# 2gunsu/monocon-pytorch

Measured on AMD Instinct MI355X. Metric: images/sec (384x1280) fwd+bwd, higher is better.
Workload: dtype f32 (f16x2); 1 GPU; train step B=32/GPU 3x384x1280 (configs[2] shape, fp32 values, mode f16x2); global_batch=32, parallelism=dp1, precision_mode=f16x2

## Files before the change

### monocon-pytorch_amd/csrc/mc_train_api.hip

```cpp
#include "mc_internal.h"

#include <algorithm>
#include <cmath>
#include <cstdlib>
#include <cstring>
#include <vector>

static int check_targets(mc_handle *h, const mc_targets *t, const char *who) {
    if (!t) return fail(h, "%s: targets is NULL", who);
    const void *p[] = {t->center_heatmap_target, t->wh_target, t->offset_target, t->dim_target, t->alpha_cls_target,
                       t->alpha_offset_target, t->depth_target, t->center2kpt_offset_target, t->kpt_heatmap_target,
                       t->kpt_heatmap_offset_target, t->indices, t->indices_kpt, t->mask_target,
                       t->mask_center2kpt_offset, t->mask_kpt_heatmap_offset};
    for (size_t i = 0; i < sizeof(p) / sizeof(p[0]); ++i)
        if (!p[i]) return fail(h, "%s: targets field %d is NULL", who, (int)i);
    return 0;
}

extern "C" {

int mc_make_targets(mc_handle *h, const mc_labels *lab, int B, int max_objs, int pad_h, int pad_w, int fh, int fw,
                    const mc_targets *t, void *stream) {
    if (!h) return -1;
    if (!lab || !lab->gt_bboxes || !lab->gt_labels || !lab->gt_bboxes_3d || !lab->depths || !lab->gt_kpts_2d ||
// ... 114 lines not shown
    HIPCHK(h, mc::launch_focal_grad(preds[0], t->center_heatmap_target, (size_t)B * 3 * HW, aux + 0, grad_losses, 0, dpreds[0], st, wrt_pred));
    HIPCHK(h, mc::launch_focal_grad(preds[1], t->kpt_heatmap_target, (size_t)B * 9 * HW, aux + 1, grad_losses, 5, dpreds[1], st, wrt_pred));
    mc::GatherLossArgs g{};
    fill_gather_args(g, preds, dpreds, t, B, max_objs, (int)HW, scratch_losses, aux + 2, grad_losses);
    g.wrt_pred = wrt_pred;
    g.partial = gather_ws(h);
    HIPCHK(h, mc::launch_gathered_losses(g, 1, st));
    return 0;
}

int mc_losses_backward(mc_handle *h, const float *const preds[MC_NUM_PREDS], const mc_targets *t, int B, int max_objs,
                       int fh, int fw, const float *grad_losses, float *const dpreds[MC_NUM_PREDS], void *stream) {
    return losses_backward_impl(h, preds, t, B, max_objs, fh, fw, grad_losses, dpreds, stream, 0);
}

int mc_losses_backward_pred(mc_handle *h, const float *const preds[MC_NUM_PREDS], const mc_targets *t, int B, int max_objs,
                            int fh, int fw, const float *grad_losses, float *const dpreds[MC_NUM_PREDS], void *stream) {
    return losses_backward_impl(h, preds, t, B, max_objs, fh, fw, grad_losses, dpreds, stream, 1);
}

int mc_op_conv_wgrad(mc_handle *h, const float *const src[], const int src_channels[], int nsrc, int B, int Hin, int Win,
                     const float *dy, int Cout, int ksize, int stride, float *dw_oihw, void *stream) {
    if (!h) return -1;
    if (!src || !src_channels || !dy || !dw_oihw || nsrc < 1 || nsrc > 4) return fail(h, "mc_op_conv_wgrad: bad argument");
    if (!((ksize == 3 && (stride == 1 || stride == 2)) || (ksize == 1 && stride == 1)))
        return fail(h, "mc_op_conv_wgrad: unsupported k=%d stride=%d", ksize, stride);
    if (Cout % 4) return fail(h, "mc_op_conv_wgrad: Cout must be a multiple of 4");
    HIPCHK(h, hipSetDevice(h->device));
    hipStream_t st = static_cast<hipStream_t>(stream);
    mc::WgradArgs a{};
    int cin = 0;
    for (int i = 0; i < nsrc; ++i) {
        if (!src[i] || src_channels[i] % 16) return fail(h, "mc_op_conv_wgrad: source %d needs C %% 16 == 0", i);
        a.src[i].p = src[i]; a.src[i].C = src_channels[i];
        cin += src_channels[i];
    }
    a.nsrc = nsrc; a.B = B; a.Hin = Hin; a.Win = Win;
    a.Hout = (Hin + 2 * (ksize / 2) - ksize) / stride + 1;
    a.Wout = (Win + 2 * (ksize / 2) - ksize) / stride + 1;
    a.Cin = cin; a.Cout = Cout; a.dy = dy; a.dy_ld = Cout;
    a.prec = h->prec;
    ScratchBuf slots;
    if (h->prec == 3) {
        HIPCHK(h, slots.alloc(5 * mc::AMAX_WORDS * sizeof(unsigned)));
        unsigned *sl = slots.as<unsigned>();
        HIPCHK(h, hipMemsetAsync(sl, 0, 5 * mc::AMAX_WORDS * sizeof(unsigned), st));
        for (int i = 0; i < nsrc; ++i) {
            HIPCHK(h, mc::launch_absmax(src[i], (size_t)B * Hin * Win * src_channels[i], sl + i * mc::AMAX_WORDS, st));
            a.amax_x[i] = sl + i * mc::AMAX_WORDS;
        }
        HIPCHK(h, mc::launch_absmax(dy, (size_t)B * a.Hout * a.Wout * Cout, sl + 4 * mc::AMAX_WORDS, st));
        a.amax_dy = sl + 4 * mc::AMAX_WORDS;
    }
    mc::wgrad_plan(a, ksize, stride);
    void *part = nullptr;
    HIPCHK(h, hipMalloc(&part, mc::wgrad_partial_floats(a, ksize) * sizeof(float)));
    a.partial = static_cast<float *>(part);
    hipError_t e = mc::launch_wgrad(a, ksize, stride, dw_oihw, st);
    hipError_t e2 = hipStreamSynchronize(st);
    (void)hipFree(part);
    HIPCHK(h, e);
    HIPCHK(h, e2);
    return 0;
}

int mc_op_conv_dgrad(mc_handle *h, const float *dy, const float *weight_oihw, int B, int Hin, int Win, int CinTotal,
                     int c_off, int Cs, int Cout, int ksize, int stride, int accumulate, float *dx, void *stream) {
    if (!h) return -1;
    if (!dy || !weight_oihw || !dx) return fail(h, "mc_op_conv_dgrad: null argument");
    if (!((ksize == 3 && (stride == 1 || stride == 2)) || (ksize == 1 && stride == 1)))
        return fail(h, "mc_op_conv_dgrad: unsupported k=%d stride=%d", ksize, stride);
    if (Cout % 16 || Cs % 4 || c_off < 0 || c_off + Cs > CinTotal) return fail(h, "mc_op_conv_dgrad: bad channel arguments");
    if (stride == 2 && ((Hin | Win) & 1)) return fail(h, "mc_op_conv_dgrad: stride 2 needs even Hin, Win");
    HIPCHK(h, hipSetDevice(h->device));
    hipStream_t st = static_cast<hipStream_t>(stream);
    const int Ho = (Hin + 2 * (ksize / 2) - ksize) / stride + 1, Wo = (Win + 2 * (ksize / 2) - ksize) / stride + 1;
    const int CsP = mc::conv_coutp(Cs), pieces = h->prec == 2 ? 3 : (h->prec == 3 ? 2 : 1);
    const int nclass = stride == 2 ? 4 : 1;
    std::vector<void *> tmp;
    hipError_t e = hipSuccess;
    ScratchBuf slots;
    unsigned *sl = nullptr;
    if (h->prec == 3) {
        HIPCHK(h, slots.alloc((mc::AMAX_WORDS + 1) * sizeof(unsigned)));
        sl = slots.as<unsigned>();
        HIPCHK(h, hipMemsetAsync(sl, 0, (mc::AMAX_WORDS + 1) * sizeof(unsigned), st));
        HIPCHK(h, mc::launch_absmax(dy, (size_t)B * Ho * Wo * Cout, sl, st));
        HIPCHK(h, mc::launch_absmax(weight_oihw, (size_t)Cout * CinTotal * ksize * ksize, sl + mc::AMAX_WORDS, st, true));
    }
    for (int cls = 0; cls < nclass && e == hipSuccess; ++cls) {
        const int cid = stride == 2 ? cls : -1;
        const int py = cls >> 1, px = cls & 1;
        const int taps = stride == 2 ? (1 + py) * (1 + px) : ksize * ksize;
        const size_t pn = (size_t)taps * Cout * CsP;
        void *panel = nullptr, *panel16 = nullptr;
        if (hipMalloc(&panel, pn * 4) != hipSuccess) { e = hipErrorOutOfMemory; break; }
        tmp.push_back(panel);
        (void)hipMemsetAsync(panel, 0, pn * 4, st);
        e = mc::launch_pack_conv_w_dgrad(weight_oihw, Cout, CinTotal, ksize, c_off, Cs, CsP, Cout, cid, static_cast<float *>(panel), st);
        if (e != hipSuccess) break;
        if (h->prec >= 1 && Cout % 32 == 0) {
            if (hipMalloc(&panel16, pn * 2 * pieces) != hipSuccess) { e = hipErrorOutOfMemory; break; }
            tmp.push_back(panel16);
            (void)hipMemsetAsync(panel16, 0, pn * 2 * pieces, st);
            e = mc::launch_pack_conv_w_dgrad_bf16(weight_oihw, Cout, CinTotal, ksize, c_off, Cs, CsP, Cout, cid, pieces, panel16, st,
                                                  sl ? sl + mc::AMAX_WORDS : nullptr);
            if (e != hipSuccess) break;
        }
        mc::ConvArgs d{};
        d.nsrc = 1; d.src[0].p = dy; d.src[0].C = Cout;
// ... 81 lines not shown
```

### monocon-pytorch_amd/csrc/mc_train_plan.hip

```cpp
#include <atomic>
#include <deque>
#include <functional>

#include "mc_internal.h"

using namespace mc;

namespace {

using Fn = std::function<int(mc_handle *, hipStream_t)>;

struct PlanSwitches {
    long long lazy_z;
    long long lazy_min;
    long long lazy_feat;
    long long zbits;
    long long grad_pool;
    long long grad_pool_cool;
    long long head_dx_fuse;
    long long dgrad_s2_thin;
    long long stem_fuse;
    long long bm_epilogue;
    long long wres_bwd;
    long long dual_stream;
    int side_sync_lo = 0, side_sync_hi = 0;
    bool plan_debug = false;
};
const struct { const char *name; long long PlanSwitches::*field; long long def; } SWITCH_TABLE[] = {
    {"MONOCON_HIP_LAZY_Z", &PlanSwitches::lazy_z, 3},
    {"MONOCON_HIP_LAZY_MIN", &PlanSwitches::lazy_min, 900000},
    {"MONOCON_HIP_LAZY_FEAT", &PlanSwitches::lazy_feat, 0},
    {"MONOCON_HIP_ZBITS", &PlanSwitches::zbits, 1},
    {"MONOCON_HIP_GRAD_POOL", &PlanSwitches::grad_pool, 1},
    {"MONOCON_HIP_GRAD_POOL_COOL", &PlanSwitches::grad_pool_cool, 2},
    {"MONOCON_HIP_HEAD_DX_FUSE", &PlanSwitches::head_dx_fuse, 1},
    {"MONOCON_HIP_DGRAD_S2_THIN", &PlanSwitches::dgrad_s2_thin, 1},
    {"MONOCON_HIP_STEM_FUSE", &PlanSwitches::stem_fuse, 1},
    {"MONOCON_HIP_BM_EPILOGUE", &PlanSwitches::bm_epilogue, 1},
    {"MONOCON_HIP_WRES_BWD", &PlanSwitches::wres_bwd, 0},
    {"MONOCON_HIP_DUAL_STREAM", &PlanSwitches::dual_stream, 1},
};
PlanSwitches read_switches() {
    PlanSwitches sw{};
    std::string changed;
    for (const auto &d : SWITCH_TABLE) {
        const char *e = std::getenv(d.name);
        sw.*d.field = e ? std::atoll(e) : d.def;
        if (sw.*d.field != d.def) changed += std::string(" ") + d.name + "=" + std::to_string(sw.*d.field);
    }
    if (const char *e = std::getenv("MONOCON_HIP_SIDE_SYNC")) {
        if (std::sscanf(e, "%d:%d", &sw.side_sync_lo, &sw.side_sync_hi) != 2) sw.side_sync_lo = sw.side_sync_hi = 0;
        if (sw.side_sync_lo < sw.side_sync_hi) changed += std::string(" MONOCON_HIP_SIDE_SYNC=") + e;
    }
    sw.plan_debug = std::getenv("MONOCON_HIP_PLAN_DEBUG") != nullptr;
    if (sw.plan_debug && !changed.empty()) fprintf(stderr, "[plan] switches off their defaults:%s\n", changed.c_str());
    return sw;
}

struct PoolBwdArgs {
    const float *x, *dout, *la, *lb;
    float *dx, *stats;
    int B, H, W, C, acc;
};

struct LastWriter {
    enum Kind { NONE, DGRAD_CONV, POOL_BWD, DECONV_BWD } kind = NONE;
    union {
        ConvArgs *conv;
        PoolBwdArgs *pool;
        float **deconv_stats;
    };
    LastWriter() : conv(nullptr) {}
    LastWriter(ConvArgs *c) : kind(c ? DGRAD_CONV : NONE), conv(c) {}
    LastWriter(PoolBwdArgs *p) : kind(p ? POOL_BWD : NONE), pool(p) {}
    LastWriter(float **s) : kind(s ? DECONV_BWD : NONE), deconv_stats(s) {}
};

struct TNode {
    Tensor t;
    float *g = nullptr;
    bool ginit = false, needs_grad = true;
    LastWriter last;
    const float *la = nullptr, *lb = nullptr;
    bool lrelu = true;
};

struct PackJob {
    const float *w;
    int Cout, CinTotal, k, c_off, Cs, CsP, CoutPad;
    int cls;
    float *dst;
    void *dst16;
    unsigned *amax;
// ... 411 lines not shown
                    HIPCHK(hh, launch_dgrad_s2_thin(dyp, B, Hd, Wd, Cd, w_master, CinTotal, c_off, gp, acc, dmax, wmax, st));
                    return 0;
                });
                wrote(srcnode);
                return;
            }
            for (int cls = 0; cls < 4; ++cls) {
                const int py = cls >> 1, px = cls & 1;
                ConvArgs d = dgrad_conv(cls);
                const int ld = sn.t.C;
                d.out = sn.g + ((size_t)py * sn.t.W + px) * ld; d.out_ld = ld;
                d.o_px = 2 * ld; d.o_row = 2 * sn.t.W * ld; d.o_img = sn.t.H * sn.t.W * ld;
                if (sn.ginit) { d.res = d.out; d.res_ld = ld; d.r_px = d.o_px; d.r_row = d.o_row; d.r_img = d.o_img; }
                const int kcode = (1 + py) * 10 + (1 + px);
                const int kk = kcode == 11 ? 1 : kcode;
                d.cfg = ts->ok ? mc_choose_conv_cfg(h, d, kk, 1) : CFG_128x32;
                push_bwd([=](mc_handle *hh, hipStream_t st) { HIPCHK(hh, launch_conv(d, kk, 1, st)); return 0; });
            }
            wrote(srcnode);
            return;
        }
        ConvArgs d = dgrad_conv(-1);
        d.out = sn.g; d.out_ld = sn.t.C;
        if (sn.ginit) { d.res = sn.g; d.res_ld = sn.t.C; }
        if (dy.H != sn.t.H || dy.W != sn.t.W) { ts->ok = false; h->err = "train plan: dgrad shape mismatch"; }
        d.cfg = ts->ok ? mc_choose_conv_cfg(h, d, ks, 1) : CFG_128x32;
        if (sw.wres_bwd < 2) d.cfg &= ~CFG_WRES;
        ts->dgrads.push_back(d);
        ConvArgs *dp = &ts->dgrads.back();
        push_bwd([=](mc_handle *hh, hipStream_t st) { HIPCHK(hh, launch_conv(*dp, ks, 1, st)); return 0; });
        wrote(srcnode, (d.cfg == CFG_SMALL && !conv_thin_ok(d, ks, 1)) ? nullptr : dp);
    }

    int emit_wgrad(const std::vector<int> &srcs, const Tensor &dy, int dy_ld, int Cout, int ks, int stride, float *dw) {
        WgradArgs a{};
        a.nsrc = (int)srcs.size();
        auto fill = [&] {
            int cin = 0;
            for (int i = 0; i < a.nsrc; ++i) {
                fill_src(a.src[i], srcs[i]);
                a.amax_x[i] = ts->nodes[srcs[i]].t.amax;
                cin += a.src[i].C;
            }
            return cin;
        };
        for (int s_ : srcs)
            if (ts->nodes[s_].la && !ts->nodes[s_].lrelu) materialise(s_);
        int cin = fill();
        a.amax_dy = dy.amax;
        const Tensor &s0 = ts->nodes[srcs[0]].t;
        a.B = s0.B; a.Hin = s0.H; a.Win = s0.W; a.Hout = dy.H; a.Wout = dy.W; a.Cin = cin; a.Cout = Cout;
        a.dy = dy.p; a.dy_ld = dy_ld;
        a.prec = h->prec;
        wgrad_plan(a, ks, stride);
        bool any_lazy = false;
        for (int i = 0; i < a.nsrc; ++i) any_lazy |= a.src[i].la != nullptr;
        if (any_lazy && !wgrad_lazy_capable(a, ks, stride)) {
            for (int s_ : srcs) materialise(s_);
            fill();
        }
        a.partial = alloc(wgrad_partial_floats(a, ks));
        return push_bwd([=](mc_handle *hh, hipStream_t st) { HIPCHK(hh, launch_wgrad(a, ks, stride, dw, st)); return 0; }, ON_SIDE);
    }

    struct BnBwd { Tensor dy; float *coef; bool affine_skipped; };
    BnBwd bn_backward(const Rec &r, const std::string &bn, bool caller_forms_dy = false) {
        TNode &zn = ts->nodes[r.z];
        Tensor dy = r.y;
        dy.p = zn.g;
        dy.amax = slot();
        unsigned *dymax = dy.amax;
        const int B = r.y.B, C = r.y.C, rows = r.y.H * r.y.W;
        const float *yp = r.y.p, *gz = zn.g, *zp = zn.t.p, *gamma = P(bn + ".weight", C), *mean = r.mean, *rstd = r.rstd;
        float *dg = G(bn + ".weight", C), *db = G(bn + ".bias", C), *dyp = dy.p;
        float *coef = alloc((size_t)C * 4);
        const int relu = r.relu ? ((r.res < 0 && r.ca && r.cb) ? 2 : 1) : 0;
        const float *fa = r.ca, *fb = r.cb;
        float *gres = nullptr;
        int gmode = 0;
        if (r.res >= 0 && ts->nodes[r.res].needs_grad) {
            gres = g_acquire(r.res);
            gmode = ts->nodes[r.res].ginit ? 2 : 1;
            wrote(r.res);
        }
        const double n = (double)B * rows;
        auto step = [&](float *partial, int nbp, int cstride, bool reduce, bool affine) {
            double *fold = fold_scratch(nbp, C);
            const int arelu = reduce ? relu : 0;
            const float *aa = reduce ? fa : nullptr, *ab = reduce ? fb : nullptr;
            push_bwd([=](mc_handle *hh, hipStream_t st) {
                if (reduce) HIPCHK(hh, launch_chan_reduce(yp, gz, zp, nullptr, B, rows, C, 1, relu, partial, C, st, fa, fb));
                HIPCHK(hh, launch_bn_bwd_finalize(partial, nbp, cstride, n, C, gamma, mean, rstd, dg, db, coef, st, fold));
                if (affine)
                    HIPCHK(hh, launch_affine_bwd(gz, zp, yp, coef, B, (size_t)rows, C, 0, arelu, dyp, gres, gmode, st, aa, ab, nullptr,
                                                 nullptr, dymax));
                return 0;
            });
            return BnBwd{dy, coef, !affine};
        };
        const LastWriter last = zn.last;
        ConvArgs *lc = last.kind == LastWriter::DGRAD_CONV ? last.conv : nullptr;
        if (sw.bm_epilogue == 0 || (sw.bm_epilogue > 1 && r.y.H * r.y.W > sw.bm_epilogue)) lc = nullptr;
        if (sw.plan_debug)
            fprintf(stderr, "[plan] bn_backward %-40s %4d ch %4dx%-4d relu %d res %d last-writer-conv %d\n", bn.c_str(), C, r.y.H,
                    r.y.W, relu, r.res >= 0, lc != nullptr);
        if (lc && lc->out == zn.g && lc->Cout == C && lc->out_ld == C && lc->Hout == r.y.H && lc->Wout == r.y.W && !lc->stats) {
// ... 608 lines not shown
```

### monocon-pytorch_amd/csrc/train.h

```cpp
#pragma once
#include <hip/hip_runtime.h>
#include <stdint.h>
#include <vector>

#include "conv_mfma.h"

namespace mc {

struct TargetArgs {
    const float *gt_bboxes, *gt_labels, *gt_bboxes_3d, *depths, *gt_kpts_2d, *gt_kpts_valid, *mask;
    int B, max_objs, num_kpt, num_classes, fh, fw;
    float h_ratio, w_ratio;
    float *center_heatmap, *kpt_heatmap;
    float *wh, *offset, *dim, *alpha_cls, *alpha_offset, *depth, *c2k, *kho;
    long long *indices, *indices_kpt;
    uint8_t *mask_target;
    float *mask_c2k, *mask_kho;
};
hipError_t launch_make_targets(const TargetArgs &a, hipStream_t st);

hipError_t launch_focal(const float *p, const float *t, size_t n, float *partial, float *loss_out, float *aux,
                        hipStream_t st);
hipError_t launch_focal_grad(const float *p, const float *t, size_t n, const float *aux, const float *gscale, int gidx,
                             float *dlogit, hipStream_t st, int wrt_pred = 0);
// ... 104 lines not shown
                                const float *wpk, float *din,
                                float *stats = nullptr);

hipError_t launch_pack_conv_w_dgrad(const float *w, int Cout, int CinTotal, int k, int c_off, int Cs, int CsP, int CoutPad,
                                    int cls, float *dst, hipStream_t st);
hipError_t launch_dpred_pack(const float *const dpred[10], int ld, int B, int HW, float *out, hipStream_t st);
hipError_t launch_dpred_pack_user(const float *const dpred[10], const float *const pred[10], const float *const grad[10], int ld,
                                  int B, int HW, float *out, hipStream_t st);
struct AttnTrainArgs {
    const float *stats;
    int chunks, stat_ld, B, HW;
    double *stats64;
    float *rm[9], *rv[9];
    long long *nbt[9];
    const float *att_w[9], *att_g[9], *att_b[9];
    float *att_rm[9], *att_rv[9];
    long long *att_nbt[9];
    const float *weight_[9], *bias_[9];
    float *sv_inst;
    float *mu_r;
    float *bn10;
    float *that, *yatt;
    float *gamma_p;
    float *scale, *shift;
};
struct AttnGradPtrs { float *d_weight_[9], *d_bias_[9], *d_att_w[9], *d_att_g[9], *d_att_b[9]; };
hipError_t launch_attn_train_fwd(const AttnTrainArgs &a, hipStream_t st);
hipError_t launch_attn_train_bwd(const AttnTrainArgs &a, const float *partial, int rb_per_img, const AttnGradPtrs &gp,
                                 float *coef, hipStream_t st);
hipError_t launch_head_bwd(const float *draw, int ld, const float *z, const float *x, const float *w1, int B, int HW,
                           int blocks, float *d, float *dw_partial, float *red_partial, hipStream_t st,
                           const float *scale = nullptr, const float *shift = nullptr);
hipError_t launch_head_dx(const float *draw, int ld, const float *x, const float *w1, const float *coef, int B, int HW, int blocks,
                          float *dx, float *csum, float *csum_out, unsigned *amax, hipStream_t st, const float *scale,
                          const float *shift);
hipError_t launch_splitk_reduce(const float *partial, int ksplit, int T, int Cout, int Cin, float *dw, hipStream_t st);
int stem_wgrad_blocks(int B, int H, int W);
hipError_t launch_stem_wgrad(const float *img, const float *dy, int B, int H, int W, float *partial, float *dw,
                             hipStream_t st, const unsigned *img_amax = nullptr, const unsigned *dy_amax = nullptr,
                             const float *y = nullptr, const float *coef = nullptr, const unsigned *y_amax = nullptr);

struct WgradArgs {
    ConvSrc src[4];
    int nsrc;
    int B, Hin, Win, Hout, Wout, Cin, Cout;
    const float *dy;
    int dy_ld;
    float *partial;
    int ksplit, n_tiles, c_tiles, ppr, ppi, groups_per_img;
    int small;
    int prec;
    int pb;
    int pipe;
    const unsigned *amax_x[4], *amax_dy;
};
void wgrad_plan(WgradArgs &a, int ks, int stride);
size_t wgrad_partial_floats(const WgradArgs &a, int ks);
hipError_t launch_wgrad(const WgradArgs &a, int ks, int stride, float *dw_oihw, hipStream_t st);
bool wgrad_lazy_capable(const WgradArgs &a, int ks, int stride);
bool wgrad_bf16_ok(const WgradArgs &a, int ks, int stride);
hipError_t launch_wgrad_bf16(const WgradArgs &a, int ks, int stride, int WN, int WC, hipStream_t st);
int wgrad_bf16_patches(int prec);
int wgrad_pipe_tile(const WgradArgs &a, int ks, int stride);
void wgrad_pipe_plan(WgradArgs &a, int tile);
hipError_t launch_wgrad_pipe(const WgradArgs &a, int ks, hipStream_t st);
bool wgrad_thin_ok(const WgradArgs &a, int ks, int stride);
hipError_t launch_wgrad_thin(const WgradArgs &a, hipStream_t st);

}
```

### monocon-pytorch_amd/csrc/wgrad_mfma.hip

```cpp
#include <algorithm>
#include <cstdlib>
#include "conv_mfma.h"
#include "train.h"

namespace mc {

template <int KS, int S, int WN, int WC>
struct WgCfg {
    static constexpr int PB = 2;
    static constexpr int NB = 32 * WN, CB = 32 * WC;
    static constexpr int NT = 64 * WN * WC;
    static constexpr int PAD = KS / 2;
    static constexpr int IH = 3 * S + KS, IW = 7 * S + KS, NPIX = IH * IW;
    static constexpr int CBP = CB + 4, NBP = NB + 4;
    static constexpr int LDS_FLOATS = PB * NPIX * CBP + PB * 32 * NBP;
    static constexpr size_t LDS_BYTES = sizeof(float) * LDS_FLOATS;
};

template <int KS, int S, int WN, int WC>
__global__ __launch_bounds__(64 * WN * WC, 2) void wgrad_mfma_kernel(const WgradArgs a) {
    using Cfg = WgCfg<KS, S, WN, WC>;
    constexpr int PB = Cfg::PB, NB = Cfg::NB, CB = Cfg::CB, NT = Cfg::NT, PAD = Cfg::PAD;
    constexpr int IW = Cfg::IW, NPIX = Cfg::NPIX, CBP = Cfg::CBP, NBP = Cfg::NBP;
    constexpr int T = KS * KS;
// ... 282 lines not shown
    for (int e = tid; e < 9 * NTN * 4 * 64; e += 256) {
        const int l = e & 63, idx = e >> 6;
        const int q = idx & 3, nt = (idx >> 2) % NTN, t = (idx >> 2) / NTN;
        const int n = nt * 16 + 4 * (l >> 4) + q, c = l & 15;
        a.partial[(((size_t)blockIdx.x * 9 + t) * COUT + n) * CIN + c] = red[idx][l];
    }
}

static bool wgrad_is_small(const WgradArgs &a, int ks, int stride) {
    return ks == 3 && a.nsrc == 1 && a.Cin == 16 && (a.Cout == 16 || a.Cout == 32) && a.dy_ld == a.Cout &&
           (stride == 1 || stride == 2) && a.Wout % 4 == 0 && a.Wout >= 8 &&
           a.Hout == (a.Hin + 2 - 3) / stride + 1 && a.Wout == (a.Win + 2 - 3) / stride + 1;
}

template <int KS, int S, int WN, int WC>
static hipError_t launch_wg(WgradArgs a, hipStream_t st) {
    using Cfg = WgCfg<KS, S, WN, WC>;
    auto kern = wgrad_mfma_kernel<KS, S, WN, WC>;
    static DynLdsOnce attr_set;
    static const size_t lds_req = [] {
#ifdef MC_DEBUG_HOOKS
        const char *e = std::getenv("MONOCON_HIP_WGRAD_LDS_KB");
        const size_t pad = e ? (size_t)std::atoi(e) * 1024 : 0;
        return pad > Cfg::LDS_BYTES ? pad : (size_t)Cfg::LDS_BYTES;
#else
        return (size_t)Cfg::LDS_BYTES;
#endif
    }();
    {
        const hipError_t e = attr_set.ensure(reinterpret_cast<const void *>(kern), (int)(lds_req));
        if (e != hipSuccess) return e;
    }
    hipLaunchKernelGGL(kern, dim3(a.ksplit * a.n_tiles * a.c_tiles), dim3(Cfg::NT), lds_req, st, a);
    return hipGetLastError();
}

static void wgrad_shape(const WgradArgs &a, int *WN, int *WC) {
    bool src64 = true;
    for (int i = 0; i < a.nsrc; ++i) src64 = src64 && (a.nsrc == 1 || a.src[i].C % 64 == 0);
    if (a.Cout > 32 && a.Cin > 32 && src64) { *WN = 2; *WC = 2; }
    else if (a.Cout > 64) { *WN = 4; *WC = 1; }
    else if (a.Cout > 32) { *WN = 2; *WC = 1; }
    else { *WN = 1; *WC = 1; }
}
static bool wgrad_sources_ok(const WgradArgs &a) {
    for (int i = 0; i < a.nsrc; ++i)
        if (a.src[i].C % 4 || (a.nsrc > 1 && a.src[i].C % 32)) return false;
    return a.dy_ld % 4 == 0;
}

void wgrad_plan(WgradArgs &a, int ks, int stride) {
    a.small = 0;
    a.pipe = 0;
    if (wgrad_is_small(a, ks, stride)) {
        a.small = 1;
        const int rows = a.B * a.Hout;
        a.ksplit = std::min(rows / 4 > 0 ? rows / 4 : 1, 1024);
        a.n_tiles = a.c_tiles = 1;
        a.ppr = a.ppi = a.groups_per_img = 0;
        return;
    }
    if (const int tile = wgrad_pipe_tile(a, ks, stride)) { wgrad_pipe_plan(a, tile); return; }
    int WN, WC;
    wgrad_shape(a, &WN, &WC);
    a.n_tiles = (a.Cout + 32 * WN - 1) / (32 * WN);
    a.c_tiles = (a.Cin + 32 * WC - 1) / (32 * WC);
    a.ppr = (a.Wout + 7) / 8;
    a.ppi = a.ppr * ((a.Hout + 3) / 4);
    a.pb = (a.prec >= 1 && wgrad_bf16_ok(a, ks, stride)) ? wgrad_bf16_patches(a.prec) : 2;
    a.groups_per_img = (a.ppi + a.pb - 1) / a.pb;
    const long long G = (long long)a.B * a.groups_per_img;
    const char *eb = std::getenv("MONOCON_HIP_WGRAD_BLOCKS");
    const int target = eb ? std::atoi(eb) : 512;
    int ks_ = target * 4 / (WN * WC) / (a.n_tiles * a.c_tiles);
    if (ks_ < 1) ks_ = 1;
    if (ks_ > G) ks_ = (int)G;
    a.ksplit = ks_;
}
size_t wgrad_partial_floats(const WgradArgs &a, int ks) { return (size_t)a.ksplit * ks * ks * a.Cout * a.Cin; }

bool wgrad_lazy_capable(const WgradArgs &a, int ks, int stride) {
    if (a.prec != 3) return false;
    if (a.pipe) return a.pipe == 4;
    if (a.small) return wgrad_thin_ok(a, ks, stride) || (ks == 3 && stride == 2 && a.Cout == 32 && a.nsrc == 1);
    return wgrad_sources_ok(a) && wgrad_bf16_ok(a, ks, stride);
}

hipError_t launch_wgrad(const WgradArgs &a, int ks, int stride, float *dw_oihw, hipStream_t st) {
    for (int i = 0; i < a.nsrc; ++i)
        if (a.src[i].la && !wgrad_lazy_capable(a, ks, stride)) return hipErrorInvalidValue;
    prof_last = {2, 2.0 * a.B * a.Hout * a.Wout * (double)a.Cout * a.Cin * ks * ks,
                 4.0 * ((double)a.B * a.Hin * a.Win * a.Cin + (double)a.B * a.Hout * a.Wout * a.Cout + (double)ks * ks * a.Cin * a.Cout)};
    hipError_t e = hipErrorInvalidValue;
    if (a.pipe) {
        e = launch_wgrad_pipe(a, ks, st);
    } else if (a.small && wgrad_thin_ok(a, ks, stride)) {
        e = launch_wgrad_thin(a, st);
    } else if (a.small && a.src[0].la) {
        if (stride == 2 && a.Cout == 32 && a.src[0].lb) hipLaunchKernelGGL((wgrad_small_kernel<2, 2, true>), dim3(a.ksplit), dim3(256), 0, st, a);
        else return hipErrorInvalidValue;
        e = hipGetLastError();
    } else if (a.small) {
        if (stride == 1 && a.Cout == 16) hipLaunchKernelGGL((wgrad_small_kernel<1, 1>), dim3(a.ksplit), dim3(256), 0, st, a);
        else if (stride == 1) hipLaunchKernelGGL((wgrad_small_kernel<1, 2>), dim3(a.ksplit), dim3(256), 0, st, a);
        else if (a.Cout == 16) hipLaunchKernelGGL((wgrad_small_kernel<2, 1>), dim3(a.ksplit), dim3(256), 0, st, a);
        else hipLaunchKernelGGL((wgrad_small_kernel<2, 2>), dim3(a.ksplit), dim3(256), 0, st, a);
        e = hipGetLastError();
    } else {
        int WN, WC;
        wgrad_shape(a, &WN, &WC);
        if (!wgrad_sources_ok(a)) return hipErrorInvalidValue;
        if (a.prec >= 1 && wgrad_bf16_ok(a, ks, stride)) {
            e = launch_wgrad_bf16(a, ks, stride, WN, WC, st);
        } else {
#define WG_DISPATCH(KS_, S_)                                                     \
    if (WN == 4) e = launch_wg<KS_, S_, 4, 1>(a, st);                            \
    else if (WN == 2 && WC == 2) e = launch_wg<KS_, S_, 2, 2>(a, st);            \
    else if (WN == 2) e = launch_wg<KS_, S_, 2, 1>(a, st);                       \
    else e = launch_wg<KS_, S_, 1, 1>(a, st);
        if (ks == 3 && stride == 1) { WG_DISPATCH(3, 1) }
        else if (ks == 3 && stride == 2) { WG_DISPATCH(3, 2) }
        else if (ks == 1 && stride == 1) { WG_DISPATCH(1, 1) }
#undef WG_DISPATCH
        }
    }
    if (e != hipSuccess) return e;
    return launch_splitk_reduce(a.partial, a.ksplit, ks * ks, a.Cout, a.Cin, dw_oihw, st);
}

hipError_t launch_splitk_reduce(const float *partial, int ksplit, int T, int Cout, int Cin, float *dw, hipStream_t st) {
    if (Cin % 4) return hipErrorInvalidValue;
    const size_t total = (size_t)T * Cout * Cin;
#define WR_LAUNCH(KL_)                                                                                              \
    hipLaunchKernelGGL((wgrad_reduce_kernel<KL_>), dim3((unsigned)((total / 4 + 256 / KL_ - 1) / (256 / KL_))), \
                       dim3(256), 0, st, partial, ksplit, T, Cout, Cin, dw)
    if (ksplit >= 2048 && total <= 65536) WR_LAUNCH(64);
    else if (ksplit >= 32) WR_LAUNCH(16);
    else if (ksplit >= 4) WR_LAUNCH(4);
    else WR_LAUNCH(1);
#undef WR_LAUNCH
    return hipGetLastError();
}

}
```

Measured before the change: 672.7 images/sec.

## Add streaming MFMA wgrad kernel for 1x1 stride-1 convolutions

Adds a new weight-gradient kernel for 1x1 stride-1 convolutions in fp16-split mode. It streams pixel groups through double-buffered LDS tiles with a three-slot register prefetch and a split-f16 (hi/lo) MFMA product, and fuses the lazy BN/activation transform into the load path. It is enabled by default in the training plan (stream=1), replacing the previous bf16/pipe path for these layers. An optional mode 2 does an in-kernel ticketed tree reduction of the k-split partials. The cost is extra partial buffer space and the precision of the three-product f16 split.

New measurement: 676.0 images/sec, median of 6. No clear change (+0.5%).

```diff
diff --git a/monocon-pytorch_amd/csrc/mc_train_api.hip b/monocon-pytorch_amd/csrc/mc_train_api.hip
--- a/monocon-pytorch_amd/csrc/mc_train_api.hip
+++ b/monocon-pytorch_amd/csrc/mc_train_api.hip
@@ -190,10 +190,20 @@
         HIPCHK(h, mc::launch_absmax(dy, (size_t)B * a.Hout * a.Wout * Cout, sl + 4 * mc::AMAX_WORDS, st));
         a.amax_dy = sl + 4 * mc::AMAX_WORDS;
     }
+    {
+        const char *e = std::getenv("MONOCON_HIP_WGRAD_STREAM");
+        a.stream = e ? std::atoi(e) : 1;
+    }
     mc::wgrad_plan(a, ksize, stride);
     void *part = nullptr;
-    HIPCHK(h, hipMalloc(&part, mc::wgrad_partial_floats(a, ksize) * sizeof(float)));
+    const size_t part_floats = mc::wgrad_partial_floats(a, ksize);
+    HIPCHK(h, hipMalloc(&part, part_floats * sizeof(float)));
     a.partial = static_cast<float *>(part);
+    if (a.stream == 2) {
+        const size_t off = mc::wgrad_stream_ticket_offset(a);
+        const hipError_t ez = hipMemsetAsync(a.partial + off, 0, (part_floats - off) * sizeof(float), st);
+        if (ez != hipSuccess) { (void)hipFree(part); HIPCHK(h, ez); }
+    }
     hipError_t e = mc::launch_wgrad(a, ksize, stride, dw_oihw, st);
     hipError_t e2 = hipStreamSynchronize(st);
     (void)hipFree(part);
diff --git a/monocon-pytorch_amd/csrc/mc_train_plan.hip b/monocon-pytorch_amd/csrc/mc_train_plan.hip
--- a/monocon-pytorch_amd/csrc/mc_train_plan.hip
+++ b/monocon-pytorch_amd/csrc/mc_train_plan.hip
@@ -23,6 +23,7 @@
     long long bm_epilogue;
     long long wres_bwd;
     long long dual_stream;
+    long long wgrad_stream;
     int side_sync_lo = 0, side_sync_hi = 0;
     bool plan_debug = false;
 };
@@ -39,6 +40,7 @@
     {"MONOCON_HIP_BM_EPILOGUE", &PlanSwitches::bm_epilogue, 1},
     {"MONOCON_HIP_WRES_BWD", &PlanSwitches::wres_bwd, 0},
     {"MONOCON_HIP_DUAL_STREAM", &PlanSwitches::dual_stream, 1},
+    {"MONOCON_HIP_WGRAD_STREAM", &PlanSwitches::wgrad_stream, 1},
 };
 PlanSwitches read_switches() {
     PlanSwitches sw{};
@@ -556,6 +558,7 @@
         a.B = s0.B; a.Hin = s0.H; a.Win = s0.W; a.Hout = dy.H; a.Wout = dy.W; a.Cin = cin; a.Cout = Cout;
         a.dy = dy.p; a.dy_ld = dy_ld;
         a.prec = h->prec;
+        a.stream = (int)sw.wgrad_stream;
         wgrad_plan(a, ks, stride);
         bool any_lazy = false;
         for (int i = 0; i < a.nsrc; ++i) any_lazy |= a.src[i].la != nullptr;
diff --git a/monocon-pytorch_amd/csrc/train.h b/monocon-pytorch_amd/csrc/train.h
--- a/monocon-pytorch_amd/csrc/train.h
+++ b/monocon-pytorch_amd/csrc/train.h
@@ -180,6 +180,7 @@
     int prec;
     int pb;
     int pipe;
+    int stream;
     const unsigned *amax_x[4], *amax_dy;
 };
 void wgrad_plan(WgradArgs &a, int ks, int stride);
@@ -192,6 +193,11 @@
 int wgrad_pipe_tile(const WgradArgs &a, int ks, int stride);
 void wgrad_pipe_plan(WgradArgs &a, int tile);
 hipError_t launch_wgrad_pipe(const WgradArgs &a, int ks, hipStream_t st);
+int wgrad_stream_tile(const WgradArgs &a, int ks, int stride);
+void wgrad_stream_plan(WgradArgs &a, int tile);
+size_t wgrad_stream_partial_floats(const WgradArgs &a);
+size_t wgrad_stream_ticket_offset(const WgradArgs &a);
+hipError_t launch_wgrad_stream(const WgradArgs &a, float *dw_oihw, hipStream_t st);
 bool wgrad_thin_ok(const WgradArgs &a, int ks, int stride);
 hipError_t launch_wgrad_thin(const WgradArgs &a, hipStream_t st);
 
diff --git a/monocon-pytorch_amd/csrc/wgrad_mfma.hip b/monocon-pytorch_amd/csrc/wgrad_mfma.hip
--- a/monocon-pytorch_amd/csrc/wgrad_mfma.hip
+++ b/monocon-pytorch_amd/csrc/wgrad_mfma.hip
@@ -358,6 +358,8 @@
 void wgrad_plan(WgradArgs &a, int ks, int stride) {
     a.small = 0;
     a.pipe = 0;
+    const int want_stream = a.stream;
+    a.stream = 0;
     if (wgrad_is_small(a, ks, stride)) {
         a.small = 1;
         const int rows = a.B * a.Hout;
@@ -367,6 +369,9 @@
         return;
     }
     if (const int tile = wgrad_pipe_tile(a, ks, stride)) { wgrad_pipe_plan(a, tile); return; }
+    a.stream = want_stream;
+    if (const int tile = wgrad_stream_tile(a, ks, stride)) { wgrad_stream_plan(a, tile); return; }
+    a.stream = 0;
     int WN, WC;
     wgrad_shape(a, &WN, &WC);
     a.n_tiles = (a.Cout + 32 * WN - 1) / (32 * WN);
@@ -383,10 +388,14 @@
     if (ks_ > G) ks_ = (int)G;
     a.ksplit = ks_;
 }
-size_t wgrad_partial_floats(const WgradArgs &a, int ks) { return (size_t)a.ksplit * ks * ks * a.Cout * a.Cin; }
+size_t wgrad_partial_floats(const WgradArgs &a, int ks) {
+    if (a.stream) return wgrad_stream_partial_floats(a);
+    return (size_t)a.ksplit * ks * ks * a.Cout * a.Cin;
+}
 
 bool wgrad_lazy_capable(const WgradArgs &a, int ks, int stride) {
     if (a.prec != 3) return false;
+    if (a.stream) return true;
     if (a.pipe) return a.pipe == 4;
     if (a.small) return wgrad_thin_ok(a, ks, stride) || (ks == 3 && stride == 2 && a.Cout == 32 && a.nsrc == 1);
     return wgrad_sources_ok(a) && wgrad_bf16_ok(a, ks, stride);
@@ -398,7 +407,11 @@
     prof_last = {2, 2.0 * a.B * a.Hout * a.Wout * (double)a.Cout * a.Cin * ks * ks,
                  4.0 * ((double)a.B * a.Hin * a.Win * a.Cin + (double)a.B * a.Hout * a.Wout * a.Cout + (double)ks * ks * a.Cin * a.Cout)};
     hipError_t e = hipErrorInvalidValue;
-    if (a.pipe) {
+    if (a.stream) {
+        if (ks != 1 || stride != 1) return hipErrorInvalidValue;
+        e = launch_wgrad_stream(a, dw_oihw, st);
+        if (a.stream == 2) return e;
+    } else if (a.pipe) {
         e = launch_wgrad_pipe(a, ks, st);
     } else if (a.small && wgrad_thin_ok(a, ks, stride)) {
         e = launch_wgrad_thin(a, st);
diff --git a/monocon-pytorch_amd/csrc/wgrad_stream.hip b/monocon-pytorch_amd/csrc/wgrad_stream.hip
--- /dev/null
+++ b/monocon-pytorch_amd/csrc/wgrad_stream.hip
@@ -0,0 +1,320 @@
+#include <algorithm>
+#include <cstdlib>
+#include "conv_mfma.h"
+#include "train.h"
+
+namespace mc {
+
+typedef _Float16 ws16x8 __attribute__((ext_vector_type(8)));
+template <int V> struct WsInt { static constexpr int value = V; };
+
+constexpr int WS_FAN = 16;
+constexpr int WS_MAX_SLICES = WS_FAN * WS_FAN;
+
+template <int WN>
+struct WgStreamCfg {
+    static constexpr int CB = 128, NB = 32 * WN, NT = 256, GP = 32;
+    static constexpr int CH = 2 * GP + 48;
+    static constexpr int X_PLANE = CB * CH, D_PLANE = NB * CH;
+    static constexpr int BUF = 2 * (X_PLANE + D_PLANE);
+    static constexpr int LZ_BYTES = 2 * (CB / 4) * 16;
+    static constexpr size_t LDS_BYTES = 2 * BUF + LZ_BYTES;
+    static_assert(LDS_BYTES <= 160 * 1024, "two tile buffers per CU");
+};
+
+__device__ __forceinline__ int ws_skew(int channel) { return ((channel >> 4) & 3) * 16; }
+__device__ __forceinline__ int ws_lane_chan(int li) { return ((li & 15) >= 4 && (li & 15) < 12) ? (li ^ 16) : li; }
+__device__ __forceinline__ void ws_split_pair(float x0, float x1, float s, unsigned &hi, unsigned &lo) {
+    unsigned h, l;
+    asm("v_fma_mixlo_f16 %0, %1, %2, 0" : "=v"(h) : "v"(x0), "v"(s));
+    asm("v_fma_mixhi_f16 %0, %1, %2, 0" : "+v"(h) : "v"(x1), "v"(s));
+    asm("v_fma_mixlo_f16 %0, %1, %2, -%3 op_sel_hi:[0,0,1]" : "=v"(l) : "v"(x0), "v"(s), "v"(h));
+    asm("v_fma_mixhi_f16 %0, %1, %2, -%3 op_sel:[0,0,1] op_sel_hi:[0,0,1]" : "+v"(l) : "v"(x1), "v"(s), "v"(h));
+    hi = h;
+    lo = l;
+}
+__device__ __forceinline__ void ws_barrier() { asm volatile("s_waitcnt lgkmcnt(0)\n\ts_barrier" ::: "memory"); }
+
+template <int NB, int CB>
+__device__ __forceinline__ void ws_reduce_tile(const float *src, int cnt, size_t wsz, float *dst, int n0, int c0, int Cout, int Cin) {
+    constexpr int Q = CB / 4;
+    for (int idx = threadIdx.x; idx < NB * Q; idx += 256) {
+        const int n = n0 + idx / Q, c = c0 + (idx % Q) * 4;
+        if (n >= Cout || c >= Cin) continue;
+        const float *p = src + (size_t)n * Cin + c;
+        f32x4 v[WS_FAN];
+#pragma unroll
+        for (int k = 0; k < WS_FAN; ++k) v[k] = *reinterpret_cast<const f32x4 *>(p + (size_t)(k < cnt ? k : cnt - 1) * wsz);
+        f32x4 s = v[0];
+#pragma unroll
+        for (int k = 1; k < WS_FAN; ++k)
+            if (k < cnt) { s[0] += v[k][0]; s[1] += v[k][1]; s[2] += v[k][2]; s[3] += v[k][3]; }
+        *reinterpret_cast<f32x4 *>(dst + (size_t)n * Cin + c) = s;
+    }
+}
+
+template <int WN, bool LZ>
+__global__ __launch_bounds__(256, 2) void wgrad_stream_kernel(const WgradArgs a, float *__restrict__ dw) {
+    using Cfg = WgStreamCfg<WN>;
+    constexpr int CB = Cfg::CB, NB = Cfg::NB, GP = Cfg::GP, CH = Cfg::CH, XPL = Cfg::X_PLANE, DPL = Cfg::D_PLANE, BUF = Cfg::BUF;
+    constexpr int WC = 4 / WN, TC = CB / 32 / WC;
+    extern __shared__ __attribute__((aligned(16))) unsigned char lds_raw[];
+    __shared__ int s_last;
+
+    const int tid = threadIdx.x, lane = tid & 63;
+    const int wave = __builtin_amdgcn_readfirstlane(tid >> 6);
+    const int wn = wave % WN, wc = wave / WN;
+    const int g = lane >> 5, li = lane & 31;
+    const int tiles = a.n_tiles * a.c_tiles;
+    const int bid = xcd_order(blockIdx.x, gridDim.x);
+    const int ct = __builtin_amdgcn_readfirstlane(bid % a.c_tiles);
+    const int nt = __builtin_amdgcn_readfirstlane((bid / a.c_tiles) % a.n_tiles);
+    const int ks = __builtin_amdgcn_readfirstlane(bid / tiles);
+    const int n0 = nt * NB, c0 = ct * CB;
+    const long long P = (long long)a.B * a.Hin * a.Win, G = (P + GP - 1) / GP;
+    const long long gb = G * ks / a.ksplit, ge = G * (ks + 1) / a.ksplit;
+    const long long p0 = gb * GP;
+    const int npx = __builtin_amdgcn_readfirstlane((int)((ge * GP < P ? ge * GP : P) - p0));
+    const int ngr = __builtin_amdgcn_readfirstlane((int)(ge - gb));
+
+    f32x16 acc[TC];
+#pragma unroll
+    for (int t = 0; t < TC; ++t)
+#pragma unroll
+        for (int r = 0; r < 16; ++r) acc[t][r] = 0.f;
+
+    const int blkx = wave >> 1, cblk = c0 + blkx * 64;
+    int si = 0, cbase = 0;
+    while (si + 1 < a.nsrc && cblk >= cbase + a.src[si].C) { cbase += a.src[si].C; ++si; }
+    const int Cs = a.src[si].C;
+    const int xq = tid & 15, xps = (tid & 127) >> 4;
+    const int xch = blkx * 64 + xq * 4, cs = c0 + xch - cbase;
+    const bool xc_ok = cs < Cs && c0 + xch < a.Cin;
+    constexpr int NIX = 2, NBLKD = NB / 64, NID = NBLKD, DPS = 16 / NBLKD;
+    const int blkd = NBLKD == 2 ? (wave >> 1) : 0;
+    const int dq = tid & 15, dps = (tid & (256 / NBLKD - 1)) >> 4;
+    const int dch = blkd * 64 + dq * 4;
+    const bool dn_ok = n0 + dch + 3 < a.dy_ld;
+    int x_stat[NIX], x_dst[NIX], d_stat[NID], d_dst[NID];
+#pragma unroll
+    for (int i = 0; i < NIX; ++i) {
+        const int pr = xps + 8 * i;
+        x_stat[i] = xc_ok ? (2 * pr * Cs + cs) * 4 : BUF_OOB;
+        x_dst[i] = xch * CH + ws_skew(xch) + pr * 4;
+    }
+#pragma unroll
+    for (int i = 0; i < NID; ++i) {
+        const int pr = dps + DPS * i;
+        d_stat[i] = dn_ok ? (2 * pr * a.dy_ld + n0 + dch) * 4 : BUF_OOB;
+        d_dst[i] = 2 * XPL + dch * CH + ws_skew(dch) + pr * 4;
+    }
+    const __amdgpu_buffer_rsrc_t r_x = make_rsrc(a.src[si].p + (size_t)p0 * Cs, (unsigned)npx * (unsigned)Cs * 4u);
+    const __amdgpu_buffer_rsrc_t r_d = make_rsrc(a.dy + (size_t)p0 * a.dy_ld, (unsigned)npx * (unsigned)a.dy_ld * 4u);
+    const int ex = f16_scale_exp(amax_read(a.amax_x[si])), ed = f16_scale_exp(amax_read(a.amax_dy));
+    const float x_scale = exp2i(ex), d_scale = exp2i(ed);
+
+    [[maybe_unused]] f32x4 *lz_tab = reinterpret_cast<f32x4 *>(lds_raw + 2 * BUF);
+    [[maybe_unused]] float lz_lo = 0.f;
+    if constexpr (LZ) {
+        const bool lz = a.src[si].la != nullptr;
+        lz_lo = lz ? 0.f : -__builtin_inff();
+        if ((tid & 127) < 16) {
+            f32x4 cA = {x_scale, x_scale, x_scale, x_scale}, cB = {0.f, 0.f, 0.f, 0.f};
+            if (lz && xc_ok) {
+                cA = *reinterpret_cast<const f32x4 *>(a.src[si].la + cs);
+                cB = *reinterpret_cast<const f32x4 *>(a.src[si].lb + cs);
+#pragma unroll
+                for (int j = 0; j < 4; ++j) { cA[j] *= x_scale; cB[j] *= x_scale; }
+            }
+            lz_tab[blkx * 16 + xq] = cA;
+            lz_tab[CB / 4 + blkx * 16 + xq] = cB;
+        }
+        __syncthreads();
+    }
+
+    f32x4 xv[3][NIX][2], dv[3][NID][2];
+    auto fetch = [&](int gl, auto slot_c) {
+        constexpr int slot = decltype(slot_c)::value;
+        const int gx = gl * (GP * 4) * Cs, gd = gl * (GP * 4) * a.dy_ld;
+#pragma unroll
+        for (int i = 0; i < NIX; ++i) {
+            xv[slot][i][0] = buf_load4(r_x, x_stat[i] + gx, 0);
+            xv[slot][i][1] = buf_load4(r_x, x_stat[i] + gx + Cs * 4, 0);
+        }
+#pragma unroll
+        for (int i = 0; i < NID; ++i) {
+            dv[slot][i][0] = buf_load4(r_d, d_stat[i] + gd, 0);
+            dv[slot][i][1] = buf_load4(r_d, d_stat[i] + gd + a.dy_ld * 4, 0);
+        }
+    };
+    auto put = [&](unsigned char *dst, int plane, const f32x4 v0, const f32x4 v1, float scale) {
+#pragma unroll
+        for (int j = 0; j < 4; ++j) {
+            unsigned hi, lo;
+            ws_split_pair(v0[j], v1[j], scale, hi, lo);
+            *reinterpret_cast<unsigned *>(dst + j * CH) = hi;
+            *reinterpret_cast<unsigned *>(dst + plane + j * CH) = lo;
+        }
+    };
+    auto convert = [&](int gl, unsigned char *buf, auto slot_c) {
+        constexpr int slot = decltype(slot_c)::value;
+        if constexpr (LZ) {
+            const f32x4 cA = lz_tab[blkx * 16 + xq], cB = lz_tab[CB / 4 + blkx * 16 + xq];
+#pragma unroll
+            for (int i = 0; i < NIX; ++i) {
+                const int px = gl * GP + 2 * (xps + 8 * i);
+                const float cap0 = px < npx ? __builtin_inff() : 0.f, cap1 = px + 1 < npx ? __builtin_inff() : 0.f;
+                f32x4 t0, t1;
+#pragma unroll
+                for (int j = 0; j < 4; ++j) {
+                    t0[j] = __builtin_amdgcn_fmed3f(__builtin_fmaf(xv[slot][i][0][j], cA[j], cB[j]), lz_lo, cap0);
+                    t1[j] = __builtin_amdgcn_fmed3f(__builtin_fmaf(xv[slot][i][1][j], cA[j], cB[j]), lz_lo, cap1);
+                }
+                put(buf + x_dst[i], XPL, t0, t1, 1.f);
+            }
+        } else {
+#pragma unroll
+            for (int i = 0; i < NIX; ++i) put(buf + x_dst[i], XPL, xv[slot][i][0], xv[slot][i][1], x_scale);
+        }
+#pragma unroll
+        for (int i = 0; i < NID; ++i) put(buf + d_dst[i], DPL, dv[slot][i][0], dv[slot][i][1], d_scale);
+    };
+
+    const int lc = ws_lane_chan(li);
+    const int a_off = 2 * XPL + (wn * 32 + lc) * CH + ws_skew(wn * 32 + lc) + g * 16;
+    int b_off[TC];
+#pragma unroll
+    for (int t = 0; t < TC; ++t) {
+        const int ch = (wc * TC + t) * 32 + lc;
+        b_off[t] = ch * CH + ws_skew(ch) + g * 16;
+    }
+    auto mfmas = [&](const unsigned char *buf) {
+#pragma unroll
+        for (int s = 0; s < GP / 16; ++s) {
+            ws16x8 av[2];
+#pragma unroll
+            for (int z = 0; z < 2; ++z) av[z] = *reinterpret_cast<const ws16x8 *>(buf + a_off + z * DPL + s * 32);
+#pragma unroll
+            for (int t = 0; t < TC; ++t) {
+                ws16x8 bv[2];
+#pragma unroll
+                for (int z = 0; z < 2; ++z) bv[z] = *reinterpret_cast<const ws16x8 *>(buf + b_off[t] + z * XPL + s * 32);
+                acc[t] = __builtin_amdgcn_mfma_f32_32x32x16_f16(av[1], bv[0], acc[t], 0, 0, 0);
+                acc[t] = __builtin_amdgcn_mfma_f32_32x32x16_f16(av[0], bv[1], acc[t], 0, 0, 0);
+                acc[t] = __builtin_amdgcn_mfma_f32_32x32x16_f16(av[0], bv[0], acc[t], 0, 0, 0);
+            }
+        }
+    };
+    auto step = [&](int gl, auto sc, auto sf) {
+        unsigned char *buf = lds_raw + (gl & 1) * BUF;
+        fetch(gl + 2, sf);
+        convert(gl, buf, sc);
+        ws_barrier();
+        mfmas(buf);
+    };
+
+    fetch(0, WsInt<0>{});
+    __builtin_amdgcn_sched_barrier(0);
+    fetch(1, WsInt<1>{});
+    __builtin_amdgcn_sched_barrier(0);
+    for (int g0 = 0; g0 < ngr; g0 += 3) {
+        step(g0, WsInt<0>{}, WsInt<2>{});
+        step(g0 + 1, WsInt<1>{}, WsInt<0>{});
+        step(g0 + 2, WsInt<2>{}, WsInt<1>{});
+    }
+
+    const size_t wsz = (size_t)a.Cout * a.Cin;
+#pragma unroll
+    for (int t = 0; t < TC; ++t) {
+        const int ctile = c0 + (wc * TC + t) * 32;
+        int st = 0, sb = 0;
+        while (st + 1 < a.nsrc && ctile >= sb + a.src[st].C) { sb += a.src[st].C; ++st; }
+        const float omul = exp2i(-f16_scale_exp(amax_read(a.amax_x[st]))) * exp2i(-ed);
+        const int c = ctile + lc;
+        if (c < a.Cin) {
+#pragma unroll
+            for (int r = 0; r < 16; ++r) {
+                const int n = n0 + wn * 32 + ws_lane_chan((r & 3) + 8 * (r >> 2) + 4 * g);
+                if (n < a.Cout) a.partial[((size_t)ks * a.Cout + n) * a.Cin + c] = acc[t][r] * omul;
+            }
+        }
+    }
+    if (a.stream != 2) return;
+
+    const int groups = (a.ksplit + WS_FAN - 1) / WS_FAN;
+    float *gsum = a.partial + (size_t)a.ksplit * wsz;
+    int *tk = reinterpret_cast<int *>(gsum + (size_t)groups * wsz) + (nt * a.c_tiles + ct) * (groups + 1);
+    const int grp = ks / WS_FAN, gsz = a.ksplit - grp * WS_FAN < WS_FAN ? a.ksplit - grp * WS_FAN : WS_FAN;
+    __threadfence();
+    __syncthreads();
+    if (tid == 0) s_last = atomicAdd(&tk[grp], 1) == gsz - 1;
+    __syncthreads();
+    if (!s_last) return;
+    __threadfence();
+    ws_reduce_tile<NB, CB>(a.partial + (size_t)grp * WS_FAN * wsz, gsz, wsz, groups == 1 ? dw : gsum + (size_t)grp * wsz, n0, c0,
+                           a.Cout, a.Cin);
+    if (tid == 0) atomicExch(&tk[grp], 0);
+    if (groups == 1) return;
+    __threadfence();
+    __syncthreads();
+    if (tid == 0) s_last = atomicAdd(&tk[groups], 1) == groups - 1;
+    __syncthreads();
+    if (!s_last) return;
+    __threadfence();
+    ws_reduce_tile<NB, CB>(gsum, groups, wsz, dw, n0, c0, a.Cout, a.Cin);
+    if (tid == 0) atomicExch(&tk[groups], 0);
+}
+
+int wgrad_stream_tile(const WgradArgs &a, int ks, int stride) {
+    if (!a.stream || a.prec != 3 || ks != 1 || stride != 1 || a.small) return 0;
+    if (a.Wout != a.Win || a.Hout != a.Hin || a.dy_ld % 4 || a.Cin % 4 || !a.amax_dy) return 0;
+    const long long P = (long long)a.B * a.Hin * a.Win;
+    if (P * a.dy_ld * 4 >= (1ll << 31)) return 0;
+    for (int i = 0; i < a.nsrc; ++i) {
+        if (!a.amax_x[i] || a.src[i].C % 4 || (a.nsrc > 1 && a.src[i].C % 64)) return 0;
+        if (P * a.src[i].C * 4 >= (1ll << 31)) return 0;
+    }
+    return a.Cout > 64 ? 4 : 2;
+}
+void wgrad_stream_plan(WgradArgs &a, int wn) {
+    a.small = a.pipe = 0;
+    a.pb = 1;
+    a.ppr = a.ppi = a.groups_per_img = 0;
+    a.n_tiles = (a.Cout + 32 * wn - 1) / (32 * wn);
+    a.c_tiles = (a.Cin + 127) / 128;
+    const char *eb = std::getenv("MONOCON_HIP_WGRAD_STREAM_BLOCKS");
+    const int blocks = eb ? std::atoi(eb) : 256;
+    a.ksplit = std::min(std::max(blocks / (a.n_tiles * a.c_tiles), 1), WS_MAX_SLICES);
+}
+size_t wgrad_stream_partial_floats(const WgradArgs &a) {
+    if (a.stream != 2) return (size_t)a.ksplit * a.Cout * a.Cin;
+    const size_t groups = (a.ksplit + WS_FAN - 1) / WS_FAN;
+    return (a.ksplit + groups) * (size_t)a.Cout * a.Cin + (size_t)a.n_tiles * a.c_tiles * (groups + 1);
+}
+size_t wgrad_stream_ticket_offset(const WgradArgs &a) {
+    const size_t groups = (a.ksplit + WS_FAN - 1) / WS_FAN;
+    return (a.ksplit + groups) * (size_t)a.Cout * a.Cin;
+}
+
+template <int WN, bool LZ>
+static hipError_t launch_ws(const WgradArgs &a, float *dw, hipStream_t st) {
+    using Cfg = WgStreamCfg<WN>;
+    auto kern = wgrad_stream_kernel<WN, LZ>;
+    static DynLdsOnce attr_set;
+    {
+        const hipError_t e = attr_set.ensure(reinterpret_cast<const void *>(kern), (int)Cfg::LDS_BYTES);
+        if (e != hipSuccess) return e;
+    }
+    hipLaunchKernelGGL(kern, dim3(a.ksplit * a.n_tiles * a.c_tiles), dim3(Cfg::NT), Cfg::LDS_BYTES, st, a, dw);
+    return hipGetLastError();
+}
+hipError_t launch_wgrad_stream(const WgradArgs &a, float *dw, hipStream_t st) {
+    if (a.ksplit < 1 || a.ksplit > WS_MAX_SLICES) return hipErrorInvalidValue;
+    bool lazy = false;
+    for (int i = 0; i < a.nsrc; ++i) lazy |= a.src[i].la != nullptr;
+    const int wn = a.Cout > 64 ? 4 : 2;
+    if (wn == 4) return lazy ? launch_ws<4, true>(a, dw, st) : launch_ws<4, false>(a, dw, st);
+    return lazy ? launch_ws<2, true>(a, dw, st) : launch_ws<2, false>(a, dw, st);
+}
+
+}
diff --git a/scratch/wgrad_stream_report.py b/scratch/wgrad_stream_report.py
--- /dev/null
+++ b/scratch/wgrad_stream_report.py
@@ -0,0 +1,77 @@
+#!/usr/bin/env python
+import collections
+import csv
+import os
+import re
+import sys
+
+src = sys.argv[1].rstrip("/")
+tag = os.path.basename(src)
+PX = {96: 32 * 96 * 320, 48: 32 * 48 * 160, 24: 32 * 24 * 80, 12: 32 * 12 * 40}
+LAYERS = [("level2.project 32->64 @96x320", 32, 64, 96), ("level2.root 128->64 @96x320", 128, 64, 96),
+          ("level3.project 64->128 @48x160", 64, 128, 48), ("level3.tree1.root 256->128 @48x160", 256, 128, 48),
+          ("level3.tree2.root 448->128 @48x160", 448, 128, 48), ("level4.project 128->256 @24x80", 128, 256, 24),
+          ("level4.tree1.root 512->256 @24x80", 512, 256, 24), ("level4.tree2.root 896->256 @24x80", 896, 256, 24),
+          ("level5.project 256->512 @12x40", 256, 512, 12), ("level5.root 1280->512 @12x40", 1280, 512, 12)]
+
+
+ORDER = [9, 8, 7, 6, 5, 4, 3, 2, 1, 0]
+
+
+def alg_mb(cin, cout, rows):
+    return PX[rows] * (cin + cout) * 4 / 2 ** 20
+
+
+def short(n):
+    return re.sub(r"\(.*", "", n).replace("void ", "")
+
+
+def is_1x1(name):
+    return "wgrad_stream_kernel" in name or "wgrad_bf16_kernel<1, 1," in name
+
+
+def per_position(path, counter=None):
+    seen = collections.OrderedDict()
+    for r in csv.DictReader(open(path)):
+        name = short(r["Kernel_Name"])
+        if not is_1x1(name):
+            continue
+        d = int(r["Dispatch_Id"]) if "Dispatch_Id" in r else len(seen)
+        gs, ws = (r["Grid_Size"], r["Workgroup_Size"]) if "Grid_Size" in r else (r["Grid_Size_X"], r["Workgroup_Size_X"])
+        e = seen.setdefault(d, [name, int(gs) // max(int(ws), 1), (int(r["End_Timestamp"]) - int(r["Start_Timestamp"])) / 1e3, 0.0])
+        if counter and r["Counter_Name"] == counter:
+            e[3] += float(r["Counter_Value"])
+    pos = collections.defaultdict(lambda: [None, 0, 0, 0.0, 0.0])
+    for i, d in enumerate(sorted(seen)):
+        name, blocks, us, val = seen[d]
+        p = pos[i % 10]
+        p[0], p[1] = name, blocks
+        p[2] += 1; p[3] += us; p[4] += val
+    return pos
+
+
+sq = per_position(os.path.join(src, "pmc_sq", "p_counter_collection.csv"), "SQ_VALU_MFMA_BUSY_CYCLES")
+gui = per_position(os.path.join(src, "pmc_sq", "p_counter_collection.csv"), "GRBM_GUI_ACTIVE")
+trace = per_position(os.path.join(src, "trace", "t_kernel_trace.csv"))
+fetch_csv = os.path.join(src, "pmc_fetch", "p_counter_collection.csv")
+fetch = per_position(fetch_csv, "FETCH_SIZE") if os.path.exists(fetch_csv) else {}
+with open(os.path.join("profiles", tag + "_wgrad_1x1.txt"), "w") as f:
+    f.write("# the ten 1x1 weight-gradient launches of a train step, by place in the step (scratch/wgrad_stream_report.py)\n")
+    f.write("# alone_us: under the counter pass (dispatches serialised); step_us: kernel trace, beside the main stream\n")
+    f.write("# hbm_rd_MB = 2 x FETCH_SIZE (the gfx950 note of make_profile_report.py); alg_MB = one read of X and dY\n")
+    f.write("%-3s %-42s %6s %4s %9s %8s %9s %9s %8s %7s %9s  %s\n" % ("pos", "kernel", "blocks", "n", "alone_us", "step_us", "mfma_busy", "hbm_rd_MB",
+                                                                 "alg_MB", "rd/alg", "alg_GB/s", "layer"))
+    tot_alone = tot_step = 0.0
+    for p in sorted(sq):
+        name, blocks, n = sq[p][:3]
+        rd = 2.0 * fetch[p][4] / fetch[p][2] / 1024.0 if p in fetch else float("nan")
+        alone = sq[p][3] / max(sq[p][2], 1)
+        busy = sq[p][4] / (1024.0 * gui[p][4] / 8.0) if gui[p][4] else 0.0
+        step = trace[p][3] / max(trace[p][2], 1) if p in trace else float("nan")
+        lname, ci, co, rows = LAYERS[ORDER[p]]
+        amb = alg_mb(ci, co, rows)
+        tot_alone += alone; tot_step += step
+        f.write("%-3d %-42s %6d %4d %9.1f %8.1f %9.3f %9.1f %8.1f %7.2f %9.0f  %s\n" % (p, name[:42], blocks, n, alone, step, busy, rd, amb, rd / amb,
+                                                                                   amb * 2 ** 20 / 1e3 / alone if alone else 0.0, lname))
+    f.write("# sum over the ten launches: alone %.1f us, in the step %.1f us\n" % (tot_alone, tot_step))
+print(open(os.path.join("profiles", tag + "_wgrad_1x1.txt")).read())
```
